# martende/findex

Hardware: AMD Instinct MI355X
Metric: rank_queries_per_sec (higher is better)
Workload: dtype u64

## Files before the change

### findex_amd/csrc/fmx_search4.h

```cpp
#pragma once
#include <type_traits>
#include "fmx_device.h"

namespace fmx {

constexpr int kSThreads = 256;

__device__ __forceinline__ uint32_t fetch4(const uint8_t *__restrict__ pat, uint64_t pos) {
  if (pos >= 4) {
    uint32_t d;
    __builtin_memcpy(&d, pat + pos - 4, 4);
    return __builtin_bswap32(d);
  }
  uint32_t r = 0;
  for (uint32_t j = 0; j < (uint32_t)pos; j++) r |= (uint32_t)pat[pos - 1 - j] << (8 * j);
  return r;
}


__device__ __forceinline__ uint32_t pat_chunk(const uint8_t *__restrict__ pat, const uint64_t *__restrict__ own,
                                              uint64_t end, uint32_t len, uint32_t j) {
  const uint32_t have = len > 4u * j ? len - 4u * j : 0u;
  const uint64_t pos = end - 4ull * j;
  const uint32_t back = have >= 4u ? 4u : have;
  const uint8_t *src = have ? pat + (pos - back) : reinterpret_cast<const uint8_t *>(own);
  uint32_t d;
  __builtin_memcpy(&d, src, 4);
  return __builtin_bswap32(d) >> (8u * (4u - (back ? back : 4u)));
}

#ifndef FMX_SEARCH_WAVES
#define FMX_SEARCH_WAVES 6
#endif
#ifdef FMX_SEARCHLOG
static __device__ unsigned long long g_searchlog[1u << 15][6];
#endif
#ifndef FMX_SEARCH_WAVES_G2
#define FMX_SEARCH_WAVES_G2 5
#endif
template <bool WIDE, uint32_t LAYOUT, uint32_t KT, uint32_t JT, uint32_t RW, bool R3T, bool G2 = false, bool KX = false>
__global__ __launch_bounds__(kSThreads) __attribute__((amdgpu_waves_per_eu(G2 ? FMX_SEARCH_WAVES_G2 : FMX_SEARCH_WAVES, 8))) void k_search4(DevIndex ix, const uint4 *__restrict__ ktab, const uint8_t *__restrict__ kdense,
                                                        uint32_t ksigma, const uint4 *__restrict__ kext, const uint4 *__restrict__ kovf,
                                                        const uint4 *__restrict__ jtab, const uint32_t jc,
                                                        const unsigned long long *__restrict__ r3tab, const uint8_t *__restrict__ pat,
                                                        const PatOff po,
                                                        uint64_t *__restrict__ sp_out, uint64_t *__restrict__ ep_out,
                                                        uint32_t k, unsigned long long *__restrict__ counters, const uint64_t pk_cap,
                                                        const uint32_t spin) {
  static_assert(!G2 || LAYOUT == kLayoutOneHot, "pairs of lanes serve the one-hot layout only");
  static_assert(!KX || (KT != 0 && JT == 2u && RW == 0u && LAYOUT == kLayoutOneHot), "level KT + 1 serves the kernels with pairs of row jump entries");
  constexpr int G = G2 ? 2 : Lay<LAYOUT>::G;
  constexpr uint32_t P = 64 / G;
  constexpr uint32_t RG = G2 ? 4u : (uint32_t)G;
  constexpr uint32_t R = LAYOUT == kLayoutBytes ? 2u : 1u;
#ifdef FMX_SEARCHLOG
  const unsigned long long sl_t0 = __builtin_amdgcn_s_memrealtime();
  unsigned long long sl_t1 = 0, sl_look = 0, sl_draw = 0;
  uint32_t sl_batches = 0;
#endif
  if (threadIdx.x == 0 && blockIdx.x < kCensusBlocks) {
    counters[(size_t)kCounterSlots * kCounterStride + 2u * blockIdx.x] = __builtin_amdgcn_s_memrealtime();
    if (blockIdx.x == 0) counters[(size_t)kCounterSlots * kCounterStride + 2u * kCensusBlocks] = gridDim.x;
  }
  if (spin & 0xFFFFu) {
    const unsigned long long c0 = __builtin_amdgcn_s_memrealtime();
    while (__builtin_amdgcn_s_memrealtime() - c0 < (spin & 0xFFFFu)) __builtin_amdgcn_s_sleep(32);
  }
  const uint32_t wave = (blockIdx.x * kSThreads + threadIdx.x) >> 6;
  const uint32_t nwaves = gridDim.x * (kSThreads / 64);
  const uint32_t grp = (threadIdx.x & 63) / G;
  auto load_off_raw = [&](uint64_t bt, uint64_t &v0, uint64_t &v1) {
    const uint64_t pid = bt * P + grp;
    const uint64_t *p = po.at(pid < k ? pid : (uint64_t)k - 1);
    v0 = p[0];
    v1 = p[1];
  };
  static_assert(kSThreads == 256, "one thread per symbol fills the tables in LDS");
  __shared__ uint4 s_tab[256];
  __shared__ uint8_t s_dense[KT ? 256 : 4];
  __shared__ uint16_t s_slot[KT ? 256 : 4];
  uint64_t raw0a, raw0b, raw1a, raw1b;
  {
    const uint4 sym = ix.symtab()[threadIdx.x];
    uint8_t dn = 0;
    uint16_t sl = 0;
    if (KT) { dn = kdense[threadIdx.x]; sl = ix.slot[threadIdx.x]; }
    load_off_raw(wave, raw0a, raw0b);
    load_off_raw((uint64_t)wave + nwaves, raw1a, raw1b);
    if (KT) { s_dense[threadIdx.x] = dn; s_slot[threadIdx.x] = sl; }
    s_tab[threadIdx.x] = sym;
  }
  __syncthreads();
  const LaneConst lc = lane_const<G2 ? 4 : G>();
  const uint32_t t = G2 ? (threadIdx.x & 1u) : lc.t;
  const uint32_t lane_off = t * 16;
  uint32_t steps = 0, reqs = 0;
  struct Blk { uint4 a, b; };
  auto blk_load = [&](uint64_t vb, uint32_t b1, uint32_t upto) -> Blk {
    const uint64_t at = vb + lane_off + (uint64_t)b1 * kBlockBytes;
    Blk w;
    w.a = load_line16(at);
    w.b = make_uint4(0, 0, 0, 0);
    if constexpr (G2) {
// ... 14 lines not shown
  auto gbc1 = [&](uint32_t v) -> uint32_t { if constexpr (G2) return pair_bcast<1>(v); else return group_bcast<G, 1>(v); };
  const uint32_t nbatch = (k + P - 1) / P;
  constexpr bool kPool = G2 || RW != 0u;
  const uint32_t tix_area = kPool ? (spin >> 16) & 0xFFu : 0u;
  const bool miss_none = JT != 0u && (spin >> 31) != 0u;
  uint32_t nstatic = nbatch;
  if (tix_area) {
    const uint32_t rounds = nbatch / nwaves, held = (spin >> 24) & 0xFu;
    if (rounds >= held + 2u) nstatic = (rounds - held) * nwaves;
  }
  constexpr bool kStage = LAYOUT != kLayoutBytes;
  constexpr uint32_t kStageBytes = G2 ? 2048 : 1024, kStagePad = 16;
  __shared__ __attribute__((aligned(16))) uint32_t s_pat[kSThreads / 64][2][kStage ? (kStagePad + kStageBytes + 16) / 4 : 4];
  uint32_t par = 0;
  constexpr bool kFold = (JT && RW == 0u) || RW != 0u;
  constexpr uint32_t kParkCap = RW ? 128u : (G2 ? 96u : 64u);
  __shared__ uint64_t s_park_row[kFold ? kSThreads / 64 : 1][kFold ? kParkCap : 1];
  __shared__ uint32_t s_park_pid[kFold ? kSThreads / 64 : 1][kFold ? kParkCap : 1];
  __shared__ uint32_t s_park_it[kFold ? kSThreads / 64 : 1][kFold ? kParkCap : 1];
  uint32_t npark = 0;
  constexpr uint32_t kRowsCap = 64u + P;
  __shared__ uint64_t s_rows_row[RW ? kSThreads / 64 : 1][RW ? kRowsCap : 1];
  __shared__ uint64_t s_rows_end[RW ? kSThreads / 64 : 1][RW ? kRowsCap : 1];
  __shared__ uint32_t s_rows_pid[RW ? kSThreads / 64 : 1][RW ? kRowsCap : 1];
  __shared__ uint32_t s_rows_it[RW ? kSThreads / 64 : 1][RW ? kRowsCap : 1];
  __shared__ uint32_t s_rows_len[RW ? kSThreads / 64 : 1][RW ? kRowsCap : 1];
  uint32_t nrows = 0;
  uint32_t rsteps = 0, rlooks = 0;
  auto st_out = [](auto *p, uint64_t v) { __builtin_nontemporal_store((decltype(*p + 0))v, p); };
  auto emit = [&](uint32_t q, uint64_t a, uint64_t b) {
    if (pk_cap != ~0ull) {
      unsigned long long *pk = reinterpret_cast<unsigned long long *>(sp_out);
      const uint64_t w = b - a;
      if (w >= kPackWide) {
        const unsigned long long slot = atomicAdd(pk + k, 1ull);
        if (slot < pk_cap) { pk[(uint64_t)k + 1 + 2 * slot] = q; pk[(uint64_t)k + 2 + 2 * slot] = b; }
      }
      st_out(pk + q, a | ((w < kPackWide ? w : kPackWide) << 40));
    } else {
      st_out(sp_out + q, a);
      st_out(ep_out + q, b);
    }
  };
  const uint32_t wave_in_wg = (uint32_t)__builtin_amdgcn_readfirstlane((int)(threadIdx.x >> 6));
  const uint32_t lane64 = threadIdx.x & 63u;
  const uint64_t pat_addr = (uint64_t)(uintptr_t)pat;
  auto fix_off = [&](uint64_t bt, uint64_t v0, uint64_t v1, uint64_t &e, uint32_t &len) {
    const uint64_t pid = bt * P + grp;
    const uint64_t q = pid < k ? pid : (uint64_t)k - 1;
    const uint64_t b = po.fixed ? q * po.fixed : v0;
    e = po.fixed ? (q + 1) * po.fixed : v1;
    len = pid < k ? (uint32_t)(e - b) : 0u;
  };
  struct Stage { uint4 w; uint4 w2; uint64_t base; bool ok; };
  auto stage_issue = [&](uint64_t e, uint32_t len) {
    const uint64_t b = e - len;
    const uint64_t b0 = ((uint64_t)__builtin_amdgcn_readfirstlane((int)(uint32_t)(b >> 32)) << 32) | (uint32_t)__builtin_amdgcn_readfirstlane((int)(uint32_t)b);
    const uint64_t e1 = ((uint64_t)(uint32_t)__builtin_amdgcn_readlane((int)(uint32_t)(e >> 32), 63) << 32) | (uint32_t)__builtin_amdgcn_readlane((int)(uint32_t)e, 63);
    Stage st;
    const uint64_t al = (pat_addr + b0) & ~15ull;
    const uint64_t span = pat_addr + e1 - al;
    st.ok = kStage && span <= kStageBytes;
    st.base = al - pat_addr;
    st.w = make_uint4(0, 0, 0, 0);
    if (st.ok && 16ull * lane64 < span) st.w = load_line16(al + 16u * lane64);
    st.w2 = make_uint4(0, 0, 0, 0);
    if constexpr (G2) {
      if (st.ok && 1024ull + 16ull * lane64 < span) st.w2 = load_line16(al + 1024u + 16u * lane64);
    }
    return st;
  };
  auto stage_park = [&](const Stage &st, uint32_t area) {
    if (st.ok) *reinterpret_cast<uint4 *>(s_pat[wave_in_wg][area] + (kStagePad + 16u * lane64) / 4) = st.w;
    if constexpr (G2) {
      if (st.ok) *reinterpret_cast<uint4 *>(s_pat[wave_in_wg][area] + (kStagePad + 1024u + 16u * lane64) / 4) = st.w2;
    }
  };
  constexpr uint32_t NT = KT ? KT / 4 : 1;
  struct Tail { uint32_t c[NT]; };
  uint64_t end0, end1, raw2a, raw2b;
  uint32_t len0, len1;
  uint32_t ktl = 0, jtl = 0, r3l = 0;
  fix_off(wave, raw0a, raw0b, end0, len0);
  fix_off((uint64_t)wave + nwaves, raw1a, raw1b, end1, len1);
  Stage cur = stage_issue(end0, len0);
  stage_park(cur, par);
  Tail tail_ahead;
#pragma unroll
  for (uint32_t i = 0; i < NT; i++) tail_ahead.c[i] = (!kStage && len0 > 4u * i) ? fetch4(pat, end0 - 4ull * i) : 0u;
  auto walk_parked = [&](auto last_tag) {
    constexpr bool kLast = decltype(last_tag)::value;
    while (npark) {
      const uint32_t take = npark < P ? npark : P;
      const bool actw = grp < take;
      const uint32_t slot = npark - take + (actw ? grp : 0u);
      npark -= take;
      const uint32_t wpid = actw ? s_park_pid[wave_in_wg][slot] : 0u;
      uint32_t wit = actw ? s_park_it[wave_in_wg][slot] : 0u;
      uint64_t wsp = actw ? s_park_row[wave_in_wg][slot] : 0ull;
      uint32_t wj = (uint32_t)(wsp >> 56);
      const bool wnone = wj == 0xFFu;
      const bool wkx = KX && actw && wj == 0xFEu;
      wj = (wnone || wkx) ? 0u : wj;
      wsp &= (1ull << 56) - 1;
      if constexpr (R3T && kLast) {
        while (__builtin_amdgcn_ballot_w64(actw && wj >= 3u)) {
          const bool go = actw && wj >= 3u;
          if (go) {
            wsp = r3tab[wsp] & ((1ull << 40) - 1);
            wj -= 3u;
            wit += 3u;
            steps += 3u;
          }
          r3l += (uint32_t)__builtin_popcountll(__builtin_amdgcn_ballot_w64(go && t == 0));
        }
      }
      uint64_t wep = wsp + ((actw && !wnone && !wkx) ? 1u : 0u);
      uint64_t wbegin = 0, wend = 0;
      if (actw) po.get(wpid, wbegin, wend);
      const uint32_t wlen = (uint32_t)(wend - wbegin);
      if constexpr (KX) {
        if (__builtin_amdgcn_ballot_w64(wkx)) {
          uint32_t code = 0;
#pragma unroll
          for (uint32_t j = 0; j < KT; j++) code = code * ksigma + s_dense[wkx ? pat[wend - 1 - j] : 0u];
          const uint4 xe = ktab[wkx ? code : 0u];
          if (wkx) {
            const uint64_t xsp = (((uint64_t)xe.y << 32) | xe.x) & ((1ull << 56) - 1), xep = ((uint64_t)xe.w << 32) | xe.z;
            if (xsp < xep) {
              steps += KT + 1u;
            } else {
              wsp = xsp;
              wep = xep;
              steps += xe.y >> 24;
            }
          }
          ktl += (uint32_t)__builtin_popcountll(__builtin_amdgcn_ballot_w64(wkx && t == 0));
        }
      }
      for (;;) {
        const uint32_t wrem = wlen - wit;
        if (!__builtin_amdgcn_ballot_w64(actw && wsp < wep && wrem != 0u)) break;
        const uint32_t nst = wrem < 8u ? wrem : 8u;
        uint64_t chars = 0;
        if (actw && wsp < wep) {
          if (nst == 8u) {
            uint32_t lo, hi;
            __builtin_memcpy(&lo, pat + (wend - wit - 8), 4);
            __builtin_memcpy(&hi, pat + (wend - wit - 4), 4);
            chars = ((uint64_t)__builtin_bswap32(lo) << 32) | __builtin_bswap32(hi);
          } else {
            for (uint32_t s8 = 0; s8 < nst; s8++) chars |= (uint64_t)pat[wend - wit - 1 - s8] << (8u * s8);
          }
        }
        for (uint32_t s8 = 0; s8 < 8; s8++) {
          const bool stepping = actw && wsp < wep && s8 < nst;
          if (!__builtin_amdgcn_ballot_w64(stepping)) break;
          if (stepping) {
            const uint32_t c = (uint32_t)(chars >> (8u * s8)) & 0xFFu;
            const uint4 en = s_tab[c];
            const uint64_t cfc = ((uint64_t)en.y << 32) | en.x;
            const uint64_t vb = ((uint64_t)en.w << 32) | en.z;
            if (vb > 1) {
              if (LAYOUT == kLayoutBytes) {
                const ByteRankReq q1 = byte_rank_issue(ix, (uint16_t)(vb - 2), wsp, lc);
                wsp = cfc + byte_rank_finish(q1, c, lc);
                wep = wsp + byte_match_bit(q1, c, lc);
              } else {
                uint32_t b1, m1;
                split448(wsp, b1, m1);
                const Blk w1 = blk_load(vb, b1, m1);
                wsp = cfc + blk_rank(w1, m1);
                wep = wsp + blk_bit(w1, m1);
              }
              reqs += R * RB;
            } else {
              const uint64_t r1 = cfc + ((vb == 1 && wsp > ix.eof) ? 1u : 0u);
              wep = cfc + ((vb == 1 && wep > ix.eof) ? 1u : 0u);
              wsp = r1;
            }
            steps++;
          }
        }
        wit += nst;
      }
      if (actw && t == 0) emit(wpid, wsp, wep);
    }
  };
  auto rows_phase = [&](const bool all) {
    if constexpr (RW != 0u) {
      while (nrows >= (all ? 1u : 64u)) {
        const uint32_t take = nrows < 64u ? nrows : 64u;
        const bool on = lane64 < take;
        const uint32_t slot = nrows - take + (on ? lane64 : 0u);
        nrows -= take;
        uint64_t row = on ? s_rows_row[wave_in_wg][slot] : 0ull;
        const uint64_t rend = on ? s_rows_end[wave_in_wg][slot] : 0ull;
        const uint32_t rpid = on ? s_rows_pid[wave_in_wg][slot] : 0u;
        const uint32_t rlen = on ? s_rows_len[wave_in_wg][slot] : 0u;
        uint32_t rit = on ? s_rows_it[wave_in_wg][slot] : 0u;
        bool live = on;
        while (__builtin_amdgcn_ballot_w64(live)) {
          const uint32_t rem = rlen - rit;
          bool fail = false;
          if constexpr (RW == 3u) {
            const bool tm = live && rem >= 3u;
            unsigned long long re = 0;
            uint32_t d = 0;
            if (tm) {
              re = r3tab[row];
              __builtin_memcpy(&d, pat + (rend - rit - 3), 4);
            }
            if (tm && (uint32_t)(re >> 40) == __builtin_bswap32(d << 8)) {
              rlooks++;
              row = re & ((1ull << 40) - 1);
              rit += 3;
              rsteps += 3;
            } else if (live) {
              rlooks += tm ? 1u : 0u;
              if (rem == 0u) emit(rpid, row, row + 1);
              else fail = true;
              live = false;
            }
          } else {
            const bool rm = live && rem != 0u;
            unsigned long long re = 0;
            uint32_t c = 0;
            if (rm) {
              re = r3tab[row];
              c = pat[rend - rit - 1];
            }
            const uint32_t c2 = (uint32_t)(re >> 40) & 0xFFu;
            if (rm && c == c2 && c2 != 0u) {
              rlooks++;
              row = re & ((1ull << 40) - 1);
              rit++;
              rsteps++;
            } else if (live) {
              rlooks += rm ? 1u : 0u;
              if (rem == 0u) emit(rpid, row, row + 1);
              else fail = true;
              live = false;
            }
          }
          const unsigned long long fm = __builtin_amdgcn_ballot_w64(fail);
          if (fm) {
            const uint32_t ps = npark + (uint32_t)__builtin_popcountll(fm & ((1ull << lane64) - 1ull));
            if (fail) { s_park_row[wave_in_wg][ps] = row; s_park_pid[wave_in_wg][ps] = rpid; s_park_it[wave_in_wg][ps] = rit; }
            npark += (uint32_t)__builtin_popcountll(fm);
          }
        }
      }
    }
  };
#ifdef FMX_SEARCHLOG
  sl_t1 = __builtin_amdgcn_s_memrealtime();
#endif
  uint32_t batch = wave;
  Stage nxt_stage;
  {
    auto search_one_batch = [&](auto staged_tag, auto ahead_tag) {
    constexpr bool STAGED = decltype(staged_tag)::value;
    constexpr bool AHEAD = decltype(ahead_tag)::value;
    const uint32_t pid = batch * P + grp;
    const bool act = pid < k;
    const uint64_t *own = po.at(act ? pid : 0u);
    const uint64_t end = end0;
    const uint32_t len = act ? len0 : 0u;
    const uint64_t cur_base = cur.base;
    const uint32_t *const spat = s_pat[wave_in_wg][par];
    auto chunk = [&](uint32_t j) -> uint32_t {
      if constexpr (!STAGED) {
        return pat_chunk(pat, own, end, len, j);
      } else {
        const uint32_t have = len > 4u * j ? len - 4u * j : 0u;
        const uint32_t o = have ? (uint32_t)(end - 4ull * j - cur_base) + (kStagePad - 4u) : 0u;
        const uint32_t lo = spat[o >> 2], hi = spat[(o >> 2) + 1];
        const uint32_t r = __builtin_bswap32(__builtin_amdgcn_alignbyte(hi, lo, o & 3u));
        return have >= 4u ? r : (r & ((1u << (8u * have)) - 1u));
      }
    };
    auto chars4 = [&](uint32_t at) -> uint32_t {
      const uint32_t have = len > at ? len - at : 0u;
      if constexpr (STAGED) {
        const uint32_t o = have ? (uint32_t)(end - at - cur_base) + (kStagePad - 4u) : 0u;
        const uint32_t lo = spat[o >> 2], hi = spat[(o >> 2) + 1];
        const uint32_t r = __builtin_bswap32(__builtin_amdgcn_alignbyte(hi, lo, o & 3u));
        return have >= 4u ? r : (r & ((1u << (8u * have)) - 1u));
      } else {
        uint32_t r = 0;
        if (have >= 4u) {
          uint32_t d;
          __builtin_memcpy(&d, pat + (end - at - 4), 4);
          r = __builtin_bswap32(d);
        } else {
          for (uint32_t j = 0; j < have; j++) r |= (uint32_t)pat[end - at - 1 - j] << (8u * j);
        }
        return r;
      }
    };
    Tail tailq;
#pragma unroll
    for (uint32_t i = 0; i < NT; i++) {
      if constexpr (STAGED) tailq.c[i] = chunk(i);
      else if constexpr (kStage) tailq.c[i] = len > 4u * i ? fetch4(pat, end - 4ull * i) : 0u;
      else tailq.c[i] = act ? tail_ahead.c[i] : 0u;
    }
    uint32_t ch = tailq.c[0];
    uint32_t nx = chunk(KT ? KT / 4 + 1 : 1);
    auto issue_ahead = [&]() {
      if constexpr (AHEAD) {
        nxt_stage = stage_issue(end1, len1);
        if constexpr (!kStage) {
#pragma unroll
          for (uint32_t i = 0; i < NT; i++) tail_ahead.c[i] = len1 > 4u * i ? fetch4(pat, end1 - 4ull * i) : 0u;
        }
        load_off_raw((uint64_t)batch + 2ull * nwaves, raw2a, raw2b);
      }
    };
    if (KT == 0) { issue_ahead(); if constexpr (AHEAD) stage_park(nxt_stage, par ^ 1u); }
    uint64_t sp = 0, ep = ix.n;
    bool kx_parked = false;
    auto special = [&](uint64_t cfc, uint64_t vb, uint64_t x) { return cfc + ((vb == 1 && x > ix.eof) ? 1u : 0u); };
    if (KT == 0) {
      if (len > 0) {
        const uint32_t c = ch & 0xFFu;
        const uint4 e = s_tab[c];
        const uint4 e2 = s_tab[(c + 1) & 0xFFu];
        const uint64_t cfc = ((uint64_t)e.y << 32) | e.x;
        const uint64_t vb = ((uint64_t)e.w << 32) | e.z;
        const uint64_t nxt = c == 255u ? ix.n : (((uint64_t)e2.y << 32) | e2.x);
        sp = vb > 1 ? cfc : special(cfc, vb, 0);
        ep = vb > 1 ? nxt : special(cfc, vb, ix.n);
        steps++;
      }
      ch >>= 8;
    } else {
      uint32_t code = 0;
      bool elig = act && len >= KT;
#pragma unroll
      for (uint32_t j = 0; j < KT; j++) {
        const uint32_t d = s_dense[(tailq.c[j >> 2] >> (8u * (j & 3u))) & 0xFFu];
        elig = elig && d != 0xFFu;
        code = code * ksigma + d;
      }
      bool ex = false;
      uint32_t chk = 0;
      uint32_t zcode = 0;
      if constexpr (KX) {
        chk = chunk(KT / 4);
        bool ez = elig && len > KT;
#pragma unroll
        for (uint32_t j = 1; j <= KT; j++) {
          const uint32_t d = s_dense[((j < KT ? tailq.c[j < KT ? j >> 2 : 0u] : chk) >> (8u * (j & 3u))) & 0xFFu];
          ez = ez && d != 0xFFu;
          zcode = zcode * ksigma + d;
        }
        ex = ez;
      }
      const uint4 *ksrc = ktab + (elig ? code : 0u);
      if constexpr (KX) { if (ex) ksrc = kext + 2ull * zcode + (t & 1u); }
#ifdef FMX_SEARCHLOG
      if (!sl_look) sl_look = __builtin_amdgcn_s_memrealtime();
#endif
      const uint4 ent = *ksrc;
      issue_ahead();
      if (elig && !ex) {
        sp = (((uint64_t)ent.y << 32) | ent.x) & ((1ull << 56) - 1);
        ep = ((uint64_t)ent.w << 32) | ent.z;
        steps += ent.y >> 24;
      }
      ktl += (uint32_t)__builtin_popcountll(__builtin_amdgcn_ballot_w64(elig && t == 0));
      if constexpr (AHEAD) stage_park(nxt_stage, par ^ 1u);
      if constexpr (KX) {
        if (__builtin_amdgcn_ballot_w64(ex)) {
          const uint32_t half = t & 1u, y = tailq.c[0] & 0xFFu;
          const uint32_t h1 = gbc0(ent.y);
          const bool big = ((h1 >> 8) & 0xFFu) == 0xFFu;
          uint32_t lt = 0, le = 0;
          auto count16 = [&](const uint4 &w, uint32_t from) {
#pragma unroll
            for (uint32_t b = 0; b < 16; b++) {
              const uint32_t x = ((b < 4 ? w.x : b < 8 ? w.y : b < 12 ? w.z : w.w) >> (8u * (b & 3u))) & 0xFFu;
              lt += (b >= from && x < y) ? 1u : 0u;
              le += (b >= from && x <= y) ? 1u : 0u;
            }
          };
          if (ex && !big) count16(ent, half ? 0u : 6u);
          uint32_t cnt = (h1 >> 8) & 0xFFu;
          if (__builtin_amdgcn_ballot_w64(ex && big)) {
            const uint32_t h2 = gbc0(ent.z), h3 = gbc0(ent.w);
            const uint64_t off = (h1 >> 16) | ((uint64_t)(h2 & 0xFFFFFFu) << 16);
            const uint32_t bc = (h2 >> 24) | (h3 << 8);
            if (ex && big) cnt = bc;
            for (uint32_t i = 0;; i++) {
              const bool more = ex && big && 32u * i < bc;
              if (!__builtin_amdgcn_ballot_w64(more)) break;
              uint4 w = make_uint4(~0u, ~0u, ~0u, ~0u);
              if (more && 32u * i + 16u * half < bc) w = kovf[off + 2u * i + half];
              if (more) count16(w, 0u);
              ktl += (uint32_t)__builtin_popcountll(__builtin_amdgcn_ballot_w64(more && t == 0));
            }
          }
          lt = gbc0(lt) + gbc1(lt);
          le = y == 255u ? cnt : gbc0(le) + gbc1(le);
          const uint64_t spz = gbc0(ent.x) | ((uint64_t)(h1 & 0xFFu) << 32);
          if (ex) {
            sp = spz + lt;
            ep = spz + le;
          }
          const bool kxp = ex && sp >= ep;
          const unsigned long long pm = __builtin_amdgcn_ballot_w64(kxp && t == 0);
          if (pm) {
            const uint32_t slot = npark + (uint32_t)__builtin_popcountll(pm & ((1ull << lane64) - 1ull));
            if (kxp && t == 0) { s_park_row[wave_in_wg][slot] = sp | (0xFEull << 56); s_park_pid[wave_in_wg][slot] = pid; s_park_it[wave_in_wg][slot] = KT + 1u; }
            npark += (uint32_t)__builtin_popcountll(pm);
          }
          kx_parked = kxp;
          if (ex && !kxp) steps += KT + 1u;
        }
      }
      constexpr uint32_t kWalk = KX ? KT + 1u : KT;
      if (__builtin_amdgcn_ballot_w64(act && !(KX ? ex : elig))) {
        for (uint32_t j = 0; j < kWalk; j++) {
          const bool stepping = act && (KX ? (!ex && j >= (elig ? KT : 0u)) : !elig) && j < len && sp < ep;
          if (!__builtin_amdgcn_ballot_w64(stepping)) {
// ... 4 lines not shown
            const uint32_t c = ((j < KT ? tailq.c[j < KT ? j >> 2 : 0u] : chk) >> (8u * (j & 3u))) & 0xFFu;
            const uint4 e = s_tab[c];
            if constexpr (G2) {
              const uint64_t cfc = ((uint64_t)e.y << 32) | e.x, vb = ((uint64_t)e.w << 32) | e.z;
              if (vb > 1) {
                uint32_t b1, b2, m1, m2;
                split448(sp, b1, m1);
                split448(ep, b2, m2);
                const Blk w1 = blk_load(vb, b1, b2 != b1 ? m1 : (m1 > m2 ? m1 : m2));
                Blk w2 = w1;
                if (b2 != b1) { w2 = blk_load(vb, b2, m2); reqs += RB; }
                sp = cfc + blk_rank(w1, m1);
                ep = cfc + blk_rank(w2, m2);
                reqs += RB;
              } else {
                const uint64_t r1 = cfc + ((vb == 1 && sp > ix.eof) ? 1u : 0u);
                ep = cfc + ((vb == 1 && ep > ix.eof) ? 1u : 0u);
                sp = r1;
              }
            } else {
              reqs += backward_step<WIDE, LAYOUT>(ix, c, s_slot[c], ((uint64_t)e.y << 32) | e.x, lc, sp, ep);
            }
            steps++;
          }
        }
      }
      if constexpr (KX) ch = chk >> 8;
      else ch = chunk(KT / 4);
    }
    constexpr uint32_t kIt0 = KX ? KT + 1u : (KT ? KT : 1u);
    uint32_t skip = 0;
    uint32_t cursor_it = kIt0;
    bool deferred = kx_parked;
    for (uint32_t it = kIt0;; it++) {
      bool alive = it < len && sp < ep;
      if constexpr (RW != 0u) {
        const bool hand = alive && (ep - sp) == 1 && (RW == 1u || (len - it) % RW == 0u);
        const unsigned long long hm = __builtin_amdgcn_ballot_w64(hand && t == 0);
        if (hm) {
          const uint32_t slot = nrows + (uint32_t)__builtin_popcountll(hm & ((1ull << lane64) - 1ull));
          if (hand && t == 0) {
            s_rows_row[wave_in_wg][slot] = sp; s_rows_end[wave_in_wg][slot] = end; s_rows_pid[wave_in_wg][slot] = pid;
            s_rows_it[wave_in_wg][slot] = it; s_rows_len[wave_in_wg][slot] = len;
          }
          nrows += (uint32_t)__builtin_popcountll(hm);
        }
        if (hand) {
          deferred = true;
          ep = sp;
          alive = false;
        }
      }
      if (!__builtin_amdgcn_ballot_w64(alive)) break;
      auto cursor_to = [&](uint32_t ni) {
        const uint32_t c0 = chars4(ni), a = ni & 3u;
        ch = a ? (c0 & ((1u << (8u * (4u - a))) - 1u)) : c0;
        nx = chunk((ni >> 2) + 1);
        cursor_it = ni;
      };
      auto chars12 = [&](uint32_t at, bool want, uint32_t &q0, uint32_t &q1, uint32_t &q2) {
        if constexpr (STAGED) {
          const uint32_t o = want ? (uint32_t)(end - at - cur_base) + (kStagePad - 12u) : 0u;
          const uint32_t w0 = o >> 2, sh = o & 3u;
          const uint32_t d0 = spat[w0], d1 = spat[w0 + 1], d2 = spat[w0 + 2], d3 = spat[w0 + 3];
          q0 = __builtin_bswap32(__builtin_amdgcn_alignbyte(d3, d2, sh));
          q1 = __builtin_bswap32(__builtin_amdgcn_alignbyte(d2, d1, sh));
          q2 = __builtin_bswap32(__builtin_amdgcn_alignbyte(d1, d0, sh));
        } else {
          q0 = chars4(at); q1 = chars4(at + 4u); q2 = chars4(at + 8u);
        }
      };
      const uint32_t rem = len - it;
      bool lookedup = false;
      bool park_now = false;
      uint32_t missj = 0;
      uint32_t park_ahead = 0;
      if (JT && !__builtin_amdgcn_ballot_w64(alive && (skip != 0u || (ep - sp) > (uint64_t)RG))) {
        const bool can = alive && rem >= jc;
        if (__builtin_amdgcn_ballot_w64(can)) {
          constexpr bool kPair = JT == 2u && STAGED && (G == 4 || G == 2);
          const uint64_t width = ep - sp;
          const bool single = !__builtin_amdgcn_ballot_w64(can && width != 1u);
          const uint32_t half = (kPair && single) ? (t & 1u) : 0u;
          const bool can2 = kPair && single && can && rem >= 2u * jc;
          uint32_t p0, p1, p2;
          chars12(it + (half && can2 ? jc : 0u), can, p0, p1, p2);
          const uint32_t m2 = jc > 8u ? ((1u << (8u * (jc - 8u))) - 1u) : 0u;
          bool jumped = false, pair_both = false, pair_then_miss = false;
          uint64_t rowj = 0;
          uint32_t nrows = 1;
          if (single) {
            uint4 je = make_uint4(0, 0, 0, 0);
            if (can) je = jtab[(JT == 2u ? 2ull * sp : sp) + (half && can2 ? 1u : 0u)];
            const uint32_t d0 = je.x ^ p0, d1 = je.y ^ p1, d2 = (je.z ^ p2) & m2;
            jumped = can && (d0 | d1 | d2) == 0u;
            missj = d0 ? (uint32_t)__builtin_ctz(d0) >> 3 : (d1 ? 4u + ((uint32_t)__builtin_ctz(d1) >> 3) : 8u + ((uint32_t)__builtin_ctz(d2 | 0x80000000u) >> 3));
            rowj = (uint64_t)(je.z >> 24) | ((uint64_t)je.w << 8);
            if constexpr (kPair) {
              const uint32_t ok = jumped ? 1u : 0u;
              const bool ok1 = gbc0(ok) != 0u, ok2 = can2 && gbc1(ok) != 0u;
              const uint32_t rlo1 = gbc0((uint32_t)rowj), rhi1 = gbc0((uint32_t)(rowj >> 32));
              const uint32_t rlo2 = gbc1((uint32_t)rowj), rhi2 = gbc1((uint32_t)(rowj >> 32));
              const uint32_t mj1 = gbc0(missj), mj2 = gbc1(missj);
              jumped = can && ok1;
              pair_both = ok1 && ok2;
              pair_then_miss = can2 && ok1 && !ok2;
// ... 180 lines not shown
            split448(ep, b2, m2);
            const Blk w1 = blk_load(vb, b1, b2 != b1 ? m1 : (m1 > m2 ? m1 : m2));
            Blk w2 = w1;
            if (b2 != b1) { w2 = blk_load(vb, b2, m2); reqs += RB; }
            sp = cfc + blk_rank(w1, m1);
            ep = cfc + blk_rank(w2, m2);
            reqs += RB;
          }
        } else {
          const uint64_t r1 = special(cfc, vb, sp);
          ep = special(cfc, vb, ep);
          sp = r1;
        }
        steps++;
      }
      ch >>= 8;
      if ((it & 3u) == 3u) {
        ch = nx;
        nx = chunk((it >> 2) + 2);
      }
      cursor_it = it + 1u;
    }
    if (act && t == 0 && !deferred) emit(pid, sp, ep);
    };
    auto one_batch = [&](auto ahead_tag) {
      if constexpr (kStage) {
        if (cur.ok) search_one_batch(std::true_type{}, ahead_tag);
        else search_one_batch(std::false_type{}, ahead_tag);
      } else {
        search_one_batch(std::false_type{}, ahead_tag);
      }
      if constexpr (RW != 0u) {
        if (nrows >= 64u) {
          if (npark > kParkCap - 64u) walk_parked(std::false_type{});
          rows_phase(false);
        }
      } else {
        if (kFold && npark > kParkCap - P) walk_parked(std::false_type{});
      }
    };
    for (; batch < nstatic; batch += nwaves) {
#ifdef FMX_SEARCHLOG
      sl_batches++;
#endif
      one_batch(std::true_type{});
      cur = nxt_stage;
      par ^= 1u;
      end0 = end1; len0 = len1;
      fix_off((uint64_t)batch + 2ull * nwaves, raw2a, raw2b, end1, len1);
    }
    if constexpr (kPool) {
    if (nstatic != nbatch) {
      const uint32_t groups = (nwaves + 31u) >> 5;
      const uint32_t nshards = groups < kTixShards ? groups : kTixShards;
      const uint32_t shard = (wave >> 5) % nshards;
      unsigned long long *tix = counters + (kCounterBytes + kCensusBytes + kCalibScratchBytes) / 8 +
                                ((size_t)(tix_area - 1u) * kTixShards + shard) * kTixStride;
      const uint32_t npool = nbatch - nstatic;
      const uint32_t pool = npool > shard ? (npool - shard + nshards - 1u) / nshards : 0u;
      const uint32_t mine = groups > shard ? (groups - shard + nshards - 1u) / nshards : 0u;
      const uint32_t drawers = mine * 32u - ((groups - 1u) % nshards == shard ? groups * 32u - nwaves : 0u);
      uint32_t drawn = 0;
#ifdef FMX_SEARCHLOG
      sl_draw = __builtin_amdgcn_s_memrealtime();
#endif
      if (lane64 == 0) drawn = (uint32_t)atomicAdd(tix, 1ull);
      for (;;) {
        const uint32_t tk = (uint32_t)__builtin_amdgcn_readfirstlane((int)drawn);
        if (tk >= pool) {
          if (tk == pool + drawers - 1u && lane64 == 0) atomicExch(tix, 0ull);
          break;
        }
        if (lane64 == 0) drawn = (uint32_t)atomicAdd(tix, 1ull);
        batch = nstatic + shard + nshards * tk;
#ifdef FMX_SEARCHLOG
        sl_batches++;
#endif
        {
          uint64_t a0, a1;
          load_off_raw(batch, a0, a1);
          fix_off(batch, a0, a1, end0, len0);
        }
        cur = stage_issue(end0, len0);
        stage_park(cur, par);
#pragma unroll
        for (uint32_t i = 0; i < NT; i++) tail_ahead.c[i] = (!kStage && len0 > 4u * i) ? fetch4(pat, end0 - 4ull * i) : 0u;
        one_batch(std::false_type{});
      }
    }
    }
  }
  if constexpr (RW != 0u) {
    if (npark > kParkCap - 64u) walk_parked(std::false_type{});
    rows_phase(true);
  }
#ifdef FMX_SEARCHLOG
  const unsigned long long sl_tw = __builtin_amdgcn_s_memrealtime();
#endif
  if (kFold) walk_parked(std::true_type{});
#ifdef FMX_SEARCHLOG
  const unsigned long long sl_t2 = __builtin_amdgcn_s_memrealtime();
#endif
  counters_add(counters, (t == 0 ? 2ull * steps : 0ull) + 2ull * rsteps, (t == 0 ? steps : 0u) + rsteps, t == 0 ? reqs : 0u);
  if (RW) {
    const unsigned long long rl = wave_sum((unsigned long long)rlooks);
    if ((threadIdx.x & 63u) == 0 && rl) atomicAdd(counters + (size_t)(blockIdx.x % kCounterSlots) * kCounterStride + 11, rl);
  }
#ifdef FMX_SEARCHLOG
  if ((threadIdx.x & 63u) == 0 && wave < (1u << 15)) {
    unsigned long long *e = g_searchlog[wave];
    e[0] = sl_t0; e[1] = ((sl_t1 - sl_t0) & 0xFFFFFFFFull) | ((sl_tw - sl_t0) << 32); e[2] = sl_t2; e[3] = __builtin_amdgcn_s_memrealtime() | ((unsigned long long)sl_batches << 48);
    e[4] = sl_look; e[5] = sl_draw;
  }
#endif
  if (threadIdx.x == 0 && blockIdx.x < kCensusBlocks)
    counters[(size_t)kCounterSlots * kCounterStride + 2u * blockIdx.x + 1u] = __builtin_amdgcn_s_memrealtime();
  if (KT) {
    const unsigned long long lookups = ktl;
    if ((threadIdx.x & 63u) == 0 && lookups)
      atomicAdd(counters + (size_t)(blockIdx.x % kCounterSlots) * kCounterStride + 9, lookups);
  }
  if (JT) {
    const unsigned long long lookups = jtl;
    if ((threadIdx.x & 63u) == 0 && lookups)
      atomicAdd(counters + (size_t)(blockIdx.x % kCounterSlots) * kCounterStride + 10, lookups);
  }
  if (JT && R3T) {
    const unsigned long long lookups = r3l;
    if ((threadIdx.x & 63u) == 0 && lookups)
      atomicAdd(counters + (size_t)(blockIdx.x % kCounterSlots) * kCounterStride + 11, lookups);
  }
}
struct Search4Args {
  DevIndex ix;
  const uint4 *ktab;
  const uint8_t *kdense;
  uint32_t ksigma;
  const uint4 *kext, *kovf;
  const uint4 *jtab;
  uint32_t jc;
  const unsigned long long *r3tab;
  const uint8_t *pat;
  PatOff po;
  uint64_t *sp_out, *ep_out;
  uint32_t k;
  unsigned long long *counters;
  uint64_t pk_cap;
  uint32_t spin;
};

template <bool WIDE, uint32_t LAYOUT, uint32_t KT, uint32_t JT, uint32_t RW, bool R3T, bool G2, bool KX>
void search4_launch(const Search4Args &a, int grid, hipStream_t st) {
// ... 45 lines not shown
```

Measured before the change: 565,500.

## Stage patterns via direct global-to-LDS loads and prefetch next pool batch

Pattern staging now uses global_load_lds, so bytes go straight from global memory into LDS instead of through registers and a separate LDS store, and completion is awaited with an explicit vmcnt wait. In the dynamic pool loop, a small state machine spread across the search iterations reads the next ticket, loads that batch's offsets and issues its staging load into the alternate buffer. This hides ticket, offset and stage latency between pool batches. It adds inline waitcnt asm and more complex ticket and reset logic, which could introduce correctness or ordering hazards.

Measured after the change: 546,000. 3.4% lower.

```diff
diff --git a/findex_amd/csrc/fmx_search4.h b/findex_amd/csrc/fmx_search4.h
--- a/findex_amd/csrc/fmx_search4.h
+++ b/findex_amd/csrc/fmx_search4.h
@@ -29,6 +29,9 @@
   return __builtin_bswap32(d) >> (8u * (4u - (back ? back : 4u)));
 }
 
+#ifndef FMX_SEARCH_WARM
+#define FMX_SEARCH_WARM 1
+#endif
 #ifndef FMX_SEARCH_WAVES
 #define FMX_SEARCH_WAVES 6
 #endif
@@ -169,29 +172,33 @@
     e = po.fixed ? (q + 1) * po.fixed : v1;
     len = pid < k ? (uint32_t)(e - b) : 0u;
   };
-  struct Stage { uint4 w; uint4 w2; uint64_t base; bool ok; };
-  auto stage_issue = [&](uint64_t e, uint32_t len) {
-    const uint64_t b = e - len;
-    const uint64_t b0 = ((uint64_t)__builtin_amdgcn_readfirstlane((int)(uint32_t)(b >> 32)) << 32) | (uint32_t)__builtin_amdgcn_readfirstlane((int)(uint32_t)b);
-    const uint64_t e1 = ((uint64_t)(uint32_t)__builtin_amdgcn_readlane((int)(uint32_t)(e >> 32), 63) << 32) | (uint32_t)__builtin_amdgcn_readlane((int)(uint32_t)e, 63);
+  struct Stage { uint64_t base; bool ok; };
+  auto stage_span = [&](const uint64_t b0, const uint64_t e1, uint32_t area) {
     Stage st;
     const uint64_t al = (pat_addr + b0) & ~15ull;
     const uint64_t span = pat_addr + e1 - al;
     st.ok = kStage && span <= kStageBytes;
     st.base = al - pat_addr;
-    st.w = make_uint4(0, 0, 0, 0);
-    if (st.ok && 16ull * lane64 < span) st.w = load_line16(al + 16u * lane64);
-    st.w2 = make_uint4(0, 0, 0, 0);
-    if constexpr (G2) {
-      if (st.ok && 1024ull + 16ull * lane64 < span) st.w2 = load_line16(al + 1024u + 16u * lane64);
+    if constexpr (kStage) {
+      if (st.ok) {
+        typedef __attribute__((address_space(1))) const void *gptr_t;
+        typedef __attribute__((address_space(3))) void *lptr_t;
+        const uint32_t o = 16u * lane64;
+        uint32_t *const dst = s_pat[wave_in_wg][area] + kStagePad / 4;
+        asm volatile("s_waitcnt lgkmcnt(0)" ::: "memory");
+        if (o < span) __builtin_amdgcn_global_load_lds((gptr_t)(uintptr_t)(al + o), (lptr_t)dst, 16, 0, 0);
+        if constexpr (G2) {
+          if (1024u + o < span) __builtin_amdgcn_global_load_lds((gptr_t)(uintptr_t)(al + 1024u + o), (lptr_t)(dst + 256), 16, 0, 0);
+        }
+      }
     }
     return st;
   };
-  auto stage_park = [&](const Stage &st, uint32_t area) {
-    if (st.ok) *reinterpret_cast<uint4 *>(s_pat[wave_in_wg][area] + (kStagePad + 16u * lane64) / 4) = st.w;
-    if constexpr (G2) {
-      if (st.ok) *reinterpret_cast<uint4 *>(s_pat[wave_in_wg][area] + (kStagePad + 1024u + 16u * lane64) / 4) = st.w2;
-    }
+  auto lane_first = [](uint64_t v) { return ((uint64_t)(uint32_t)__builtin_amdgcn_readfirstlane((int)(uint32_t)(v >> 32)) << 32) | (uint32_t)__builtin_amdgcn_readfirstlane((int)(uint32_t)v); };
+  auto lane_last = [](uint64_t v) { return ((uint64_t)(uint32_t)__builtin_amdgcn_readlane((int)(uint32_t)(v >> 32), 63) << 32) | (uint32_t)__builtin_amdgcn_readlane((int)(uint32_t)v, 63); };
+  auto stage_issue = [&](uint64_t e, uint32_t len, uint32_t area) { return stage_span(lane_first(e - len), lane_last(e), area); };
+  auto stage_wait = [&]() {
+    if constexpr (kStage) asm volatile("s_waitcnt vmcnt(0)" ::: "memory");
   };
   constexpr uint32_t NT = KT ? KT / 4 : 1;
   struct Tail { uint32_t c[NT]; };
@@ -200,8 +207,8 @@
   uint32_t ktl = 0, jtl = 0, r3l = 0;
   fix_off(wave, raw0a, raw0b, end0, len0);
   fix_off((uint64_t)wave + nwaves, raw1a, raw1b, end1, len1);
-  Stage cur = stage_issue(end0, len0);
-  stage_park(cur, par);
+  Stage cur = stage_issue(end0, len0, par);
+  stage_wait();
   Tail tail_ahead;
 #pragma unroll
   for (uint32_t i = 0; i < NT; i++) tail_ahead.c[i] = (!kStage && len0 > 4u * i) ? fetch4(pat, end0 - 4ull * i) : 0u;
@@ -375,6 +382,28 @@
 #endif
   uint32_t batch = wave;
   Stage nxt_stage;
+  unsigned long long *tix = nullptr;
+  uint32_t pool = 0, drawers = 0, shard = 0, nshards = 1;
+  uint32_t drawn = 0;
+  uint32_t chain = 0, nxt_tk = 0;
+  auto pool_batch = [&](uint32_t tk) { return nstatic + shard + nshards * tk; };
+  constexpr bool kWarm = kPool && kStage && FMX_SEARCH_WARM != 0;
+  auto chain_step = [&]() {
+    if constexpr (kWarm) {
+      if (chain == 1u) {
+        nxt_tk = (uint32_t)__builtin_amdgcn_readfirstlane((int)drawn);
+        chain = nxt_tk < pool ? 2u : 0u;
+        if (chain && !po.fixed) load_off_raw(pool_batch(nxt_tk), raw2a, raw2b);
+      } else if (chain == 2u) {
+        const uint64_t q0 = (uint64_t)pool_batch(nxt_tk) * P, q1 = q0 + P < k ? q0 + P : (uint64_t)k;
+        nxt_stage = stage_span(po.fixed ? q0 * po.fixed : lane_first(raw2a), po.fixed ? q1 * po.fixed : lane_last(raw2b), par ^ 1u);
+        chain = 3u;
+      } else if (chain == 3u) {
+        stage_wait();
+        chain = 0u;
+      }
+    }
+  };
   {
     auto search_one_batch = [&](auto staged_tag, auto ahead_tag) {
     constexpr bool STAGED = decltype(staged_tag)::value;
@@ -427,7 +456,7 @@
     uint32_t nx = chunk(KT ? KT / 4 + 1 : 1);
     auto issue_ahead = [&]() {
       if constexpr (AHEAD) {
-        nxt_stage = stage_issue(end1, len1);
+        nxt_stage = stage_issue(end1, len1, par ^ 1u);
         if constexpr (!kStage) {
 #pragma unroll
           for (uint32_t i = 0; i < NT; i++) tail_ahead.c[i] = len1 > 4u * i ? fetch4(pat, end1 - 4ull * i) : 0u;
@@ -435,7 +464,7 @@
         load_off_raw((uint64_t)batch + 2ull * nwaves, raw2a, raw2b);
       }
     };
-    if (KT == 0) { issue_ahead(); if constexpr (AHEAD) stage_park(nxt_stage, par ^ 1u); }
+    if (KT == 0) { issue_ahead(); if constexpr (AHEAD) stage_wait(); }
     uint64_t sp = 0, ep = ix.n;
     bool kx_parked = false;
     auto special = [&](uint64_t cfc, uint64_t vb, uint64_t x) { return cfc + ((vb == 1 && x > ix.eof) ? 1u : 0u); };
@@ -488,7 +517,8 @@
         steps += ent.y >> 24;
       }
       ktl += (uint32_t)__builtin_popcountll(__builtin_amdgcn_ballot_w64(elig && t == 0));
-      if constexpr (AHEAD) stage_park(nxt_stage, par ^ 1u);
+      if constexpr (AHEAD) stage_wait();
+      else chain_step();
       if constexpr (KX) {
         if (__builtin_amdgcn_ballot_w64(ex)) {
           const uint32_t half = t & 1u, y = tailq.c[0] & 0xFFu;
@@ -599,6 +629,9 @@
         }
       }
       if (!__builtin_amdgcn_ballot_w64(alive)) break;
+      if constexpr (!AHEAD && kWarm) {
+        if (chain && it != kIt0) chain_step();
+      }
       auto cursor_to = [&](uint32_t ni) {
         const uint32_t c0 = chars4(ni), a = ni & 3u;
         ch = a ? (c0 & ((1u << (8u * (4u - a))) - 1u)) : c0;
@@ -885,41 +918,50 @@
     if constexpr (kPool) {
     if (nstatic != nbatch) {
       const uint32_t groups = (nwaves + 31u) >> 5;
-      const uint32_t nshards = groups < kTixShards ? groups : kTixShards;
-      const uint32_t shard = (wave >> 5) % nshards;
-      unsigned long long *tix = counters + (kCounterBytes + kCensusBytes + kCalibScratchBytes) / 8 +
-                                ((size_t)(tix_area - 1u) * kTixShards + shard) * kTixStride;
+      nshards = groups < kTixShards ? groups : kTixShards;
+      shard = (wave >> 5) % nshards;
+      tix = counters + (kCounterBytes + kCensusBytes + kCalibScratchBytes) / 8 + ((size_t)(tix_area - 1u) * kTixShards + shard) * kTixStride;
       const uint32_t npool = nbatch - nstatic;
-      const uint32_t pool = npool > shard ? (npool - shard + nshards - 1u) / nshards : 0u;
+      pool = npool > shard ? (npool - shard + nshards - 1u) / nshards : 0u;
       const uint32_t mine = groups > shard ? (groups - shard + nshards - 1u) / nshards : 0u;
-      const uint32_t drawers = mine * 32u - ((groups - 1u) % nshards == shard ? groups * 32u - nwaves : 0u);
-      uint32_t drawn = 0;
+      drawers = mine * 32u - ((groups - 1u) % nshards == shard ? groups * 32u - nwaves : 0u);
 #ifdef FMX_SEARCHLOG
       sl_draw = __builtin_amdgcn_s_memrealtime();
 #endif
       if (lane64 == 0) drawn = (uint32_t)atomicAdd(tix, 1ull);
+      bool warm = false;
       for (;;) {
-        const uint32_t tk = (uint32_t)__builtin_amdgcn_readfirstlane((int)drawn);
-        if (tk >= pool) {
-          if (tk == pool + drawers - 1u && lane64 == 0) atomicExch(tix, 0ull);
-          break;
+        if (!warm) {
+          const uint32_t tk = (uint32_t)__builtin_amdgcn_readfirstlane((int)drawn);
+          if (tk >= pool) { nxt_tk = tk; break; }
+          batch = pool_batch(tk);
         }
         if (lane64 == 0) drawn = (uint32_t)atomicAdd(tix, 1ull);
-        batch = nstatic + shard + nshards * tk;
 #ifdef FMX_SEARCHLOG
         sl_batches++;
 #endif
-        {
+        if (!warm) {
           uint64_t a0, a1;
           load_off_raw(batch, a0, a1);
           fix_off(batch, a0, a1, end0, len0);
-        }
-        cur = stage_issue(end0, len0);
-        stage_park(cur, par);
+          cur = stage_issue(end0, len0, par);
+          stage_wait();
 #pragma unroll
-        for (uint32_t i = 0; i < NT; i++) tail_ahead.c[i] = (!kStage && len0 > 4u * i) ? fetch4(pat, end0 - 4ull * i) : 0u;
+          for (uint32_t i = 0; i < NT; i++) tail_ahead.c[i] = (!kStage && len0 > 4u * i) ? fetch4(pat, end0 - 4ull * i) : 0u;
+        }
+        if constexpr (kWarm) chain = 1u;
         one_batch(std::false_type{});
-      }
+        if constexpr (kWarm) {
+          while (chain) chain_step();
+          if (nxt_tk >= pool) break;
+          batch = pool_batch(nxt_tk);
+          cur = nxt_stage;
+          par ^= 1u;
+          fix_off(batch, raw2a, raw2b, end0, len0);
+          warm = true;
+        }
+      }
+      if (nxt_tk == pool + drawers - 1u && lane64 == 0) atomicExch(tix, 0ull);
     }
     }
   }
```

## Walk final parked queries per lane before regrouping for rank steps

Applied to the files above, without the earlier changes.

Adds a walk_last path for the final drain of parked queries, used by most kernel variants. All 64 lanes each take one parked query to do the per-query setup: r3 table jumps, the level KT+1 table lookup and gathering the next 8 pattern bytes. Only the queries that still need rank steps are then regrouped into G-lane groups, with their chars passed by shuffle. This is meant to keep whole waves busy on the latency-bound setup, where before only one lane per group did it. In exchange the code is larger and may use more registers, it needs extra LDS writes and reads to repark, and when more than 8 steps remain a query goes through another loop iteration.

New measurement: 580,000 before, 596,000 after (median of 6 runs). 2.8% higher.

```diff
diff --git a/findex_amd/csrc/fmx_search4.h b/findex_amd/csrc/fmx_search4.h
--- a/findex_amd/csrc/fmx_search4.h
+++ b/findex_amd/csrc/fmx_search4.h
@@ -49,6 +49,7 @@
                                                         const uint32_t spin) {
   static_assert(!G2 || LAYOUT == kLayoutOneHot, "pairs of lanes serve the one-hot layout only");
   static_assert(!KX || (KT != 0 && JT == 2u && RW == 0u && LAYOUT == kLayoutOneHot), "level KT + 1 serves the kernels with pairs of row jump entries");
+  static_assert(!KX || KT % 4u == 0u, "walk_last reads the last KT bytes of a level KT + 1 park as whole dwords");
   constexpr int G = G2 ? 2 : Lay<LAYOUT>::G;
   constexpr uint32_t P = 64 / G;
   constexpr uint32_t RG = G2 ? 4u : (uint32_t)G;
@@ -205,6 +206,30 @@
   Tail tail_ahead;
 #pragma unroll
   for (uint32_t i = 0; i < NT; i++) tail_ahead.c[i] = (!kStage && len0 > 4u * i) ? fetch4(pat, end0 - 4ull * i) : 0u;
+  auto walk_step = [&](uint32_t c, uint64_t &wsp, uint64_t &wep) {
+    const uint4 en = s_tab[c];
+    const uint64_t cfc = ((uint64_t)en.y << 32) | en.x;
+    const uint64_t vb = ((uint64_t)en.w << 32) | en.z;
+    if (vb > 1) {
+      if (LAYOUT == kLayoutBytes) {
+        const ByteRankReq q1 = byte_rank_issue(ix, (uint16_t)(vb - 2), wsp, lc);
+        wsp = cfc + byte_rank_finish(q1, c, lc);
+        wep = wsp + byte_match_bit(q1, c, lc);
+      } else {
+        uint32_t b1, m1;
+        split448(wsp, b1, m1);
+        const Blk w1 = blk_load(vb, b1, m1);
+        wsp = cfc + blk_rank(w1, m1);
+        wep = wsp + blk_bit(w1, m1);
+      }
+      reqs += R * RB;
+    } else {
+      const uint64_t r1 = cfc + ((vb == 1 && wsp > ix.eof) ? 1u : 0u);
+      wep = cfc + ((vb == 1 && wep > ix.eof) ? 1u : 0u);
+      wsp = r1;
+    }
+    steps++;
+  };
   auto walk_parked = [&](auto last_tag) {
     constexpr bool kLast = decltype(last_tag)::value;
     while (npark) {
@@ -273,31 +298,7 @@
         for (uint32_t s8 = 0; s8 < 8; s8++) {
           const bool stepping = actw && wsp < wep && s8 < nst;
           if (!__builtin_amdgcn_ballot_w64(stepping)) break;
-          if (stepping) {
-            const uint32_t c = (uint32_t)(chars >> (8u * s8)) & 0xFFu;
-            const uint4 en = s_tab[c];
-            const uint64_t cfc = ((uint64_t)en.y << 32) | en.x;
-            const uint64_t vb = ((uint64_t)en.w << 32) | en.z;
-            if (vb > 1) {
-              if (LAYOUT == kLayoutBytes) {
-                const ByteRankReq q1 = byte_rank_issue(ix, (uint16_t)(vb - 2), wsp, lc);
-                wsp = cfc + byte_rank_finish(q1, c, lc);
-                wep = wsp + byte_match_bit(q1, c, lc);
-              } else {
-                uint32_t b1, m1;
-                split448(wsp, b1, m1);
-                const Blk w1 = blk_load(vb, b1, m1);
-                wsp = cfc + blk_rank(w1, m1);
-                wep = wsp + blk_bit(w1, m1);
-              }
-              reqs += R * RB;
-            } else {
-              const uint64_t r1 = cfc + ((vb == 1 && wsp > ix.eof) ? 1u : 0u);
-              wep = cfc + ((vb == 1 && wep > ix.eof) ? 1u : 0u);
-              wsp = r1;
-            }
-            steps++;
-          }
+          if (stepping) walk_step((uint32_t)(chars >> (8u * s8)) & 0xFFu, wsp, wep);
         }
         wit += nst;
       }
@@ -366,6 +367,116 @@
             if (fail) { s_park_row[wave_in_wg][ps] = row; s_park_pid[wave_in_wg][ps] = rpid; s_park_it[wave_in_wg][ps] = rit; }
             npark += (uint32_t)__builtin_popcountll(fm);
           }
+        }
+      }
+    }
+  };
+  constexpr bool kLaneWalk = !(WIDE && JT == 1u && R3T && !G2);
+  auto walk_last = [&]() {
+    while (npark) {
+      const uint32_t take = npark < 64u ? npark : 64u;
+      const bool on = lane64 < take;
+      const uint32_t slot = npark - take + (on ? lane64 : 0u);
+      npark -= take;
+      const uint32_t wpid = on ? s_park_pid[wave_in_wg][slot] : 0u;
+      const uint32_t wit0 = on ? s_park_it[wave_in_wg][slot] : 0u;
+      uint64_t wsp = on ? s_park_row[wave_in_wg][slot] : 0ull;
+      uint32_t wj = (uint32_t)(wsp >> 56);
+      const bool wnone = wj == 0xFFu;
+      const bool wkx = KX && on && wj == 0xFEu;
+      wj = (wnone || wkx) ? 0u : wj;
+      wsp &= (1ull << 56) - 1;
+      const uint32_t n3 = R3T ? wj / 3u : 0u;
+      unsigned long long word = 0;
+      if constexpr (R3T) word = r3tab[n3 >= 1u ? wsp : 0ull];
+      const uint64_t *own = po.at(wpid);
+      const uint64_t o0 = own[0], o1 = own[1];
+      const uint32_t wit = wit0 + 3u * n3;
+      rsteps += 3u * n3;
+      if constexpr (R3T) {
+        r3l += (uint32_t)__builtin_popcountll(__builtin_amdgcn_ballot_w64(n3 >= 1u)) + (uint32_t)__builtin_popcountll(__builtin_amdgcn_ballot_w64(n3 >= 2u));
+        if (n3 >= 1u) wsp = word & ((1ull << 40) - 1);
+        word = r3tab[n3 >= 2u ? wsp : 0ull];
+      }
+      const uint64_t wbegin = po.fixed ? (uint64_t)wpid * po.fixed : o0, wend = po.fixed ? ((uint64_t)wpid + 1) * po.fixed : o1;
+      const uint32_t wlen = (uint32_t)(wend - wbegin);
+      const uint32_t wrem = (on && !wnone && !wkx) ? wlen - wit : 0u;
+      const uint32_t nst = wrem < 8u ? wrem : 8u;
+      uint64_t chars = 0;
+      {
+        const uint8_t *src = (nst != 0u && wlen >= 8u) ? pat + (wend - wit - nst) : reinterpret_cast<const uint8_t *>(own);
+        uint32_t lo, hi;
+        __builtin_memcpy(&lo, src, 4);
+        __builtin_memcpy(&hi, src + 4, 4);
+        const uint64_t v = ((uint64_t)__builtin_bswap32(lo) << 32) | __builtin_bswap32(hi);
+        if (nst != 0u && wlen >= 8u) chars = v >> (8u * (8u - nst));
+      }
+      uint64_t wep = wsp;
+      if constexpr (KX) {
+        uint32_t code = 0;
+#pragma unroll
+        for (uint32_t i = 0; i < KT / 4u; i++) {
+          uint32_t d;
+          __builtin_memcpy(&d, wkx ? pat + (wend - 4u * (i + 1u)) : reinterpret_cast<const uint8_t *>(own), 4);
+          d = __builtin_bswap32(d);
+#pragma unroll
+          for (uint32_t j = 0; j < 4u; j++) code = code * ksigma + s_dense[(d >> (8u * j)) & 0xFFu];
+        }
+        const uint4 xe = ktab[wkx ? code : 0u];
+        ktl += (uint32_t)__builtin_popcountll(__builtin_amdgcn_ballot_w64(wkx));
+        if (wkx) {
+          const uint64_t xsp = (((uint64_t)xe.y << 32) | xe.x) & ((1ull << 56) - 1), xep = ((uint64_t)xe.w << 32) | xe.z;
+          if (xsp < xep) {
+            rsteps += KT + 1u;
+          } else {
+            wsp = xsp;
+            wep = xep;
+            rsteps += xe.y >> 24;
+          }
+        }
+      }
+      if constexpr (R3T) {
+        if (n3 >= 2u) wsp = word & ((1ull << 40) - 1);
+        for (uint32_t lv = 3u; __builtin_amdgcn_ballot_w64(n3 >= lv); lv++) {
+          if (n3 >= lv) wsp = r3tab[wsp] & ((1ull << 40) - 1);
+          r3l += (uint32_t)__builtin_popcountll(__builtin_amdgcn_ballot_w64(n3 >= lv));
+        }
+      }
+      if (on && nst != 0u && wlen < 8u) {
+        for (uint32_t s8 = 0; s8 < nst; s8++) chars |= (uint64_t)pat[wend - wit - 1 - s8] << (8u * s8);
+      }
+      const bool walks = nst != 0u;
+      if (on && !walks) emit(wpid, wsp, (wnone || wkx) ? wep : wsp + 1u);
+      if (walks) {
+        s_park_row[wave_in_wg][slot] = wsp | ((uint64_t)(nst | (nst == wrem ? 16u : 0u)) << 56);
+        s_park_it[wave_in_wg][slot] = wit;
+      }
+      const unsigned long long wm = __builtin_amdgcn_ballot_w64(walks);
+      const uint32_t slot0 = npark;
+      for (uint32_t base = 0; base < take; base += P) {
+        if (((wm >> base) & ((1ull << P) - 1ull)) == 0ull) continue;
+        const bool actw = ((wm >> (base + grp)) & 1ull) != 0ull;
+        const uint32_t gslot = slot0 + base + (actw ? grp : 0u);
+        const uint64_t grow = s_park_row[wave_in_wg][gslot];
+        const uint32_t gpid = s_park_pid[wave_in_wg][gslot], git = s_park_it[wave_in_wg][gslot];
+        const uint32_t gnst = actw ? (uint32_t)(grow >> 56) & 15u : 0u;
+        const bool gfinal = ((uint32_t)(grow >> 60) & 1u) != 0u;
+        const int from = (int)(base + grp);
+        const uint64_t gchars = ((uint64_t)(uint32_t)__shfl((int)(uint32_t)(chars >> 32), from, 64) << 32) | (uint32_t)__shfl((int)(uint32_t)chars, from, 64);
+        uint64_t gsp = grow & ((1ull << 56) - 1);
+        uint64_t gep = gsp + 1u;
+        for (uint32_t s8 = 0; s8 < 8; s8++) {
+          const bool stepping = actw && gsp < gep && s8 < gnst;
+          if (!__builtin_amdgcn_ballot_w64(stepping)) break;
+          if (stepping) walk_step((uint32_t)(gchars >> (8u * s8)) & 0xFFu, gsp, gep);
+        }
+        const bool again = actw && gsp < gep && !gfinal;
+        if (actw && !again && t == 0) emit(gpid, gsp, gep);
+        const unsigned long long am = __builtin_amdgcn_ballot_w64(again && t == 0);
+        if (am) {
+          const uint32_t ps = npark + (uint32_t)__builtin_popcountll(am & ((1ull << lane64) - 1ull));
+          if (again && t == 0) { s_park_row[wave_in_wg][ps] = gsp; s_park_pid[wave_in_wg][ps] = gpid; s_park_it[wave_in_wg][ps] = git + gnst; }
+          npark += (uint32_t)__builtin_popcountll(am);
         }
       }
     }
@@ -930,7 +1041,10 @@
 #ifdef FMX_SEARCHLOG
   const unsigned long long sl_tw = __builtin_amdgcn_s_memrealtime();
 #endif
-  if (kFold) walk_parked(std::true_type{});
+  if constexpr (kFold) {
+    if constexpr (kLaneWalk) walk_last();
+    else walk_parked(std::true_type{});
+  }
 #ifdef FMX_SEARCHLOG
   const unsigned long long sl_t2 = __builtin_amdgcn_s_memrealtime();
 #endif
```
